# 0xPolygonZero/plonky2

Measured on NVIDIA H100. Metric: goldilocks_field_elements_per_s_ntt_lde_merkle, higher is better.
Workload: dtype u64

## Files before the change

### plonky2_b200/csrc/gl_ntt.cuh

```cuda
#pragma once
#include "gl_lazy.cuh"

namespace gl {

constexpr int NTT_MAX_LOG_PASS = 10;
constexpr int NTT_COL_MIN_LOG = 5;

GL_HD constexpr int ntt_r2(int log) { return log / 2; }
GL_HD constexpr int ntt_r1(int log) { return log - log / 2; }

template <int LOG>
struct PassCfg {
    static constexpr int R1 = ntt_r1(LOG), R2 = ntt_r2(LOG);
    static constexpr int E = 1 << R1, TPT = 1 << R2, NSUB = E / TPT;
    static constexpr int ROW_THREADS = (TPT * 8 < 32) ? 32 : TPT * 8;
    static constexpr int LPC = ROW_THREADS / TPT;
    static constexpr int ROW_MIN_BLOCKS = (E >= 32 ? 512 : 768) / ROW_THREADS;
    static constexpr int ROW_PITCH = TPT + 1;
    static constexpr int ROW_S_WORDS = E * ROW_PITCH;
    static constexpr int GATHER_PITCH = (1 << LOG) + 2;
    static constexpr int T = (256 / TPT) < 8 ? 8 : (256 / TPT);
    static constexpr int COL_THREADS = T * TPT;
    static constexpr int COL_MIN_BLOCKS = (E >= 32 ? 512 : 768) / COL_THREADS;
    static constexpr int COL_QPITCH = TPT * T + 8;
// ... 32 lines not shown
GL_HD void pass_step1(uint64_t* x, const uint64_t* tw, const uint64_t* uq, bool tw_full, int t) {
    using Cf = PassCfg<LOG>;
    L3 r[Cf::E];
#pragma unroll
    for (int q = 0; q < Cf::E; q++) {
        uint64_t v = x[q];
        if (uq && q) v = mul(v, uq[q]);
        r[q] = l3_from(v);
    }
    dft_lazy<Cf::R1>(r);
#pragma unroll
    for (int q = 0; q < Cf::E; q++) {
        uint64_t y = l3_norm(r[q]);
        if (Cf::R2 > 0 && (q || tw_full)) y = mul(y, tw[q * Cf::TPT + t]);
        if (Cf::R2 == 0 && tw_full) y = mul(y, tw[0]);
        x[q] = y;
    }
}
template <int LOG>
GL_HD void pass_step2(uint64_t* z) {
    using Cf = PassCfg<LOG>;
    L3 r[Cf::TPT];
#pragma unroll
    for (int j = 0; j < Cf::TPT; j++) r[j] = l3_from(z[j]);
    dft_lazy<Cf::R2>(r);
#pragma unroll
    for (int j = 0; j < Cf::TPT; j++) z[j] = l3_norm(r[j]);
}

struct ColPass {
    const uint64_t* in;
    uint64_t* out;
    size_t in_stride, out_stride;
    const uint64_t* tw;
    const uint64_t* twa;
    int log_c;
    int log_rb;
    int tw_full;
    int has_uq;
    uint64_t uq[32];
};
template <int LOG>
GL_HD void col_unit(const ColPass& cp, int blk, size_t& in_off, size_t& out_off, int& tile) {
    using Cf = PassCfg<LOG>;
    const int tiles = (1 << cp.log_c) / Cf::T;
    tile = blk % tiles;
    const int unit = blk / tiles;
    const size_t rb = (size_t)unit & (((size_t)1 << cp.log_rb) - 1), col = (size_t)unit >> cp.log_rb;
    const size_t blk_words = (size_t)1 << (LOG + cp.log_c);
    in_off = col * cp.in_stride + rb * blk_words;
    out_off = col * cp.out_stride + rb * blk_words;
}
template <int LOG>
GL_HD void col_load(const ColPass& cp, int blk, int tid, uint64_t* x) {
    using Cf = PassCfg<LOG>;
    const int tt = tid % Cf::T, t = tid / Cf::T;
    size_t in_off, out_off;
    int tile;
    col_unit<LOG>(cp, blk, in_off, out_off, tile);
    const size_t C = (size_t)1 << cp.log_c;
    const uint64_t* src = cp.in + in_off + (size_t)tile * Cf::T + tt;
#pragma unroll
    for (int q = 0; q < Cf::E; q++) x[q] = src[(size_t)(t + Cf::TPT * q) * C];
}
template <int LOG>
GL_HD void col_phase1(const ColPass& cp, uint64_t* S, int blk, int tid, uint64_t* x) {
    using Cf = PassCfg<LOG>;
    const int tt = tid % Cf::T, t = tid / Cf::T;
    size_t in_off, out_off;
    int tile;
    col_unit<LOG>(cp, blk, in_off, out_off, tile);
    const size_t C = (size_t)1 << cp.log_c;
    pass_step1<LOG>(x, cp.tw, cp.has_uq ? cp.uq : nullptr, cp.tw_full != 0, t);
    if (Cf::R2 == 0) {
        uint64_t* dst = cp.out + out_off + (size_t)tile * Cf::T + tt;
        const uint64_t* twa = cp.twa + (size_t)tile * Cf::T + tt;
#pragma unroll
        for (int q = 0; q < Cf::E; q++) dst[(size_t)q * C] = mul(x[q], twa[(size_t)q * C]);
        return;
    }
#pragma unroll
    for (int q = 0; q < Cf::E; q++) S[q * Cf::COL_QPITCH + t * Cf::T + tt] = x[q];
}
template <int LOG>
GL_HD void col_phase2_load(const uint64_t* S, int tid, uint64_t* z ) {
    using Cf = PassCfg<LOG>;
    const int tt = tid % Cf::T, t = tid / Cf::T;
#pragma unroll
    for (int m = 0; m < Cf::NSUB; m++) {
        const int q = t + Cf::TPT * m;
#pragma unroll
        for (int j = 0; j < Cf::TPT; j++) z[m * Cf::TPT + j] = S[q * Cf::COL_QPITCH + j * Cf::T + tt];
    }
}
template <int LOG>
GL_HD void col_phase2_dft(uint64_t* z) {
    using Cf = PassCfg<LOG>;
#pragma unroll
    for (int m = 0; m < Cf::NSUB; m++) pass_step2<LOG>(z + m * Cf::TPT);
}
template <int LOG>
GL_HD int col_twiddle_slot(int tid, int i) { return i * PassCfg<LOG>::COL_THREADS + tid; }
template <int LOG>
GL_HD const uint64_t* col_twiddle_src(const ColPass& cp, int blk, int tid, int i) {
    using Cf = PassCfg<LOG>;
    const int tt = tid % Cf::T, t = tid / Cf::T;
    size_t in_off, out_off;
    int tile;
    col_unit<LOG>(cp, blk, in_off, out_off, tile);
    const int m = i / Cf::TPT, j = i % Cf::TPT;
    const size_t p = (size_t)(t + Cf::TPT * m) * Cf::TPT + j;
    return cp.twa + (p << cp.log_c) + (size_t)tile * Cf::T + tt;
}
template <int LOG>
GL_HD void col_phase2_store(const ColPass& cp, int blk, int tid, const uint64_t* z, const uint64_t* tws, size_t stride_j,
                            size_t stride_m) {
    using Cf = PassCfg<LOG>;
    const int tt = tid % Cf::T, t = tid / Cf::T;
    size_t in_off, out_off;
    int tile;
    col_unit<LOG>(cp, blk, in_off, out_off, tile);
    const size_t C = (size_t)1 << cp.log_c;
    uint64_t* dst = cp.out + out_off + (size_t)tile * Cf::T + tt;
#pragma unroll
    for (int m = 0; m < Cf::NSUB; m++) {
#pragma unroll
        for (int j = 0; j < Cf::TPT; j++) {
            const int i = m * Cf::TPT + j;
            const size_t p = (size_t)(t + Cf::TPT * m) * Cf::TPT + j;
            dst[p * C] = mul(z[i], tws[m * stride_m + j * stride_j]);
        }
    }
}
template <int LOG>
GL_HD void col_phase2(const ColPass& cp, const uint64_t* S, int blk, int tid) {
    using Cf = PassCfg<LOG>;
    if (Cf::R2 == 0) return;
    uint64_t z[Cf::E];
    col_phase2_load<LOG>(S, tid, z);
    col_phase2_dft<LOG>(z);
    const size_t C = (size_t)1 << cp.log_c;
    col_phase2_store<LOG>(cp, blk, tid, z, col_twiddle_src<LOG>(cp, blk, tid, 0), C, (size_t)Cf::TPT * Cf::TPT * C);
}

enum RowMode { RM_BITREV = 0, RM_NATURAL = 1 };
struct RowPass {
    const uint64_t* in;
    uint64_t* out;
    size_t in_stride, out_stride;
    const uint64_t* tw;
    int log_r;
    int ncols;
    int tw_full;
    int has_uq;
    int reverse;
    size_t row0;
    int n_peer;
    uint64_t* out_peer[7];
    uint64_t uq[32];
};
template <int LOG, int MODE>
GL_HD bool row_line(const RowPass& rp, int blk, int l, size_t& col, size_t& prow, size_t& kbase) {
    using Cf = PassCfg<LOG>;
    const size_t L = (size_t)blk * Cf::LPC + l;
    const size_t R = (size_t)1 << rp.log_r;
    col = L >> rp.log_r;
    const size_t low = L & (R - 1);
    if (MODE == RM_BITREV) {
        prow = low;
        kbase = 0;
    } else {
        kbase = low;
        prow = rp.log_r ? (size_t)bitrev32((uint32_t)low, (uint32_t)rp.log_r) : 0;
    }
    return col < (size_t)rp.ncols;
}
template <int LOG>
GL_HD int row_blocks(const RowPass& rp) {
    using Cf = PassCfg<LOG>;
    const size_t lines = (size_t)rp.ncols << rp.log_r;
    return (int)((lines + Cf::LPC - 1) / Cf::LPC);
}
template <int LOG, int MODE>
GL_HD void row_load(const RowPass& rp, int blk, int tid, uint64_t* x) {
    using Cf = PassCfg<LOG>;
    const int l = tid / Cf::TPT, t = tid % Cf::TPT;
    size_t col, prow, kbase;
    const bool live = row_line<LOG, MODE>(rp, blk, l, col, prow, kbase);
    const uint64_t* src = rp.in + col * rp.in_stride + (prow << LOG) + t;
#pragma unroll
    for (int q = 0; q < Cf::E; q++) x[q] = live ? src[Cf::TPT * q] : 0;
}
template <int LOG, int MODE>
GL_HD void row_phase1(const RowPass& rp, uint64_t* S, int blk, int tid, uint64_t* x) {
    using Cf = PassCfg<LOG>;
    const int l = tid / Cf::TPT, t = tid % Cf::TPT;
    pass_step1<LOG>(x, rp.tw, rp.has_uq ? rp.uq : nullptr, rp.tw_full != 0, t);
    if (Cf::R2 == 0) return;
    uint64_t* Sl = S + (size_t)l * Cf::ROW_S_WORDS;
#pragma unroll
    for (int q = 0; q < Cf::E; q++) Sl[q * Cf::ROW_PITCH + t] = x[q];
}
template <int LOG>
GL_HD uint32_t row_natural_index(int q, int j) {
    using Cf = PassCfg<LOG>;
    return bitrev32((uint32_t)q, Cf::R1) + (uint32_t)Cf::E * (Cf::R2 ? bitrev32((uint32_t)j, Cf::R2) : 0u);
}
template <int LOG>
GL_HD void row_phase2_load(const uint64_t* S, int tid, int m, uint64_t* z) {
    using Cf = PassCfg<LOG>;
    const int l = tid / Cf::TPT, t = tid % Cf::TPT;
    const uint64_t* Sl = S + (size_t)l * Cf::ROW_S_WORDS;
    const int q = t + Cf::TPT * m;
#pragma unroll
    for (int j = 0; j < Cf::TPT; j++) z[j] = Sl[q * Cf::ROW_PITCH + j];
}
template <int LOG>
GL_HD void row_store_bitrev(const RowPass& rp, int blk, int tid, int m, const uint64_t* z) {
    using Cf = PassCfg<LOG>;
    const int l = tid / Cf::TPT, t = tid % Cf::TPT;
    size_t col, prow, kbase;
    if (!row_line<LOG, RM_BITREV>(rp, blk, l, col, prow, kbase)) return;
    uint64_t* dst = rp.out + col * rp.out_stride + rp.row0 + (prow << LOG);
    if constexpr (Cf::R2 == 0) {
#pragma unroll
        for (int q = 0; q < Cf::E; q++) dst[q] = canon(z[q]);
    } else {
        const int q = t + Cf::TPT * m;
        uint64_t* d = dst + (size_t)q * Cf::TPT;
#if defined(__CUDA_ARCH__)
#pragma unroll
        for (int j = 0; j < Cf::TPT; j += 2) {
            ulonglong2 v;
            v.x = canon(z[j]);
            v.y = canon(z[j + 1]);
            *reinterpret_cast<ulonglong2*>(d + j) = v;
        }
#else
        for (int j = 0; j < Cf::TPT; j++) d[j] = canon(z[j]);
#endif
    }
}
template <int LOG>
GL_HD void row_gather_write(uint64_t* G, int tid, int m, const uint64_t* z) {
    using Cf = PassCfg<LOG>;
    const int l = tid / Cf::TPT, t = tid % Cf::TPT;
    uint64_t* Gl = G + (size_t)l * Cf::GATHER_PITCH;
    if (Cf::R2 == 0) {
#pragma unroll
        for (int q = 0; q < Cf::E; q++) Gl[row_natural_index<LOG>(q, 0)] = canon(z[q]);
        return;
    }
    const int q = t + Cf::TPT * m;
#pragma unroll
    for (int j = 0; j < Cf::TPT; j++) Gl[row_natural_index<LOG>(q, j)] = canon(z[j]);
}
template <int LOG>
GL_HD void row_store_natural(const RowPass& rp, const uint64_t* G, int blk, int tid, int nthreads) {
    using Cf = PassCfg<LOG>;
    const size_t R = (size_t)1 << rp.log_r, n = R << LOG;
    for (int e = tid; e < Cf::LPC * (1 << LOG); e += nthreads) {
        int l, k2;
        if (rp.log_r) {
            l = e % Cf::LPC;
            k2 = e / Cf::LPC;
        } else {
            k2 = e & ((1 << LOG) - 1);
            l = e >> LOG;
        }
        size_t col, prow, kbase;
        if (!row_line<LOG, RM_NATURAL>(rp, blk, l, col, prow, kbase)) continue;
        size_t k = kbase + ((size_t)k2 << rp.log_r);
        if (rp.reverse) k = (n - k) & (n - 1);
        const uint64_t v = G[(size_t)l * Cf::GATHER_PITCH + k2];
        const size_t at = col * rp.out_stride + k;
        rp.out[at] = v;
        for (int p = 0; p < rp.n_peer; p++) rp.out_peer[p][at] = v;
    }
}

struct NttPlan {
    int a1, a2, b;
};
GL_HD NttPlan ntt_plan(int log_n) {
    NttPlan p{0, 0, log_n};
    if (log_n <= NTT_MAX_LOG_PASS) return p;
    if (log_n <= 2 * NTT_MAX_LOG_PASS) {
        p.b = (log_n + 1) / 2;
        p.a1 = log_n - p.b;
        return p;
    }
    p.b = (log_n + 2) / 3;
    p.a2 = (log_n - p.b + 1) / 2;
    p.a1 = log_n - p.b - p.a2;
    return p;
}


struct TableReq {
    int a, b;
    uint64_t scale, base;
};
struct NttJob {
    NttPlan pl;
    ColPass c1, c2;
    RowPass rp;
    TableReq c1_step, c1_post, c2_step, c2_post, row_step;
};
inline void ntt_make_job(int log_n, NttPlan pl, uint64_t scale, uint64_t shift, NttJob& job) {
    job = NttJob{};
    job.pl = pl;
    const bool coset = canon(shift) != 1;
    const uint64_t one = 1;
    RowPass& rp = job.rp;
    rp.log_r = log_n - pl.b;
    auto fill_uq = [](uint64_t* uq, int log_pass, uint64_t sq) {
        const int E = 1 << ntt_r1(log_pass);
        uint64_t acc = 1;
        for (int q = 0; q < E; q++, acc = mul(acc, sq)) uq[q] = canon(acc);
    };
    if (pl.a1 == 0) {
        job.row_step = TableReq{pl.b, 0, scale, coset ? shift : one};
        rp.tw_full = (canon(scale) != 1 || coset) ? 1 : 0;
        rp.has_uq = coset ? 1 : 0;
        if (coset) fill_uq(rp.uq, pl.b, pow(shift, (uint64_t)1 << ntt_r2(pl.b)));
        return;
    }
    const int c1_log = log_n - pl.a1;
    ColPass& c1 = job.c1;
    c1.log_c = c1_log;
    c1.log_rb = 0;
    job.c1_step = TableReq{pl.a1, 0, one, coset ? pow(shift, (uint64_t)1 << c1_log) : one};
    job.c1_post = TableReq{pl.a1, c1_log, one, coset ? shift : one};
    c1.tw_full = coset ? 1 : 0;
    c1.has_uq = coset ? 1 : 0;
    if (coset) fill_uq(c1.uq, pl.a1, pow(shift, ((uint64_t)1 << ntt_r2(pl.a1)) << c1_log));
    if (pl.a2) {
        ColPass& c2 = job.c2;
        c2.log_c = pl.b;
        c2.log_rb = pl.a1;
        job.c2_step = TableReq{pl.a2, 0, one, one};
        job.c2_post = TableReq{pl.a2, pl.b, one, one};
    }
    job.row_step = TableReq{pl.b, 0, scale, one};
    rp.tw_full = canon(scale) != 1 ? 1 : 0;
}
template <int LOG>
GL_HD int col_blocks(const ColPass& cp, size_t ncols) {
    return (int)((ncols << cp.log_rb) * (((size_t)1 << cp.log_c) / PassCfg<LOG>::T));
}

}
```

### plonky2_b200/csrc/gl_ntt_host.cuh

```cuda
#pragma once

template <int LOG, bool ASYNC_TW>
__global__ void __launch_bounds__(PassCfg<LOG>::COL_THREADS, PassCfg<LOG>::COL_MIN_BLOCKS) k_ntt_col(ColPass cp) {
    using Cf = PassCfg<LOG>;
    extern __shared__ __align__(16) u64 smem[];
    u64* tw_s = smem;
    u64* S = smem + (1 << LOG);
    u64* mbar = S + Cf::COL_S_WORDS;
    tma_table_issue(tw_s, cp.tw, (uint32_t)((1 << LOG) * 8), mbar);
    u64 x[Cf::E];
    col_load<LOG>(cp, blockIdx.x, threadIdx.x, x);
    __syncthreads();
    ColPass c2 = cp;
    c2.tw = tw_s;
    tma_table_wait(mbar);
    col_phase1<LOG>(c2, S, blockIdx.x, threadIdx.x, x);
    if (Cf::R2 == 0) return;
    __syncthreads();
    if (!ASYNC_TW) {
        col_phase2<LOG>(c2, S, blockIdx.x, threadIdx.x);
        return;
    }
    col_phase2_load<LOG>(S, threadIdx.x, x);
    __syncthreads();
#pragma unroll
    for (int i = 0; i < Cf::E; i++) {
        const u64* src = col_twiddle_src<LOG>(cp, blockIdx.x, threadIdx.x, i);
        asm volatile("cp.async.ca.shared.global [%0], [%1], 8;" ::"r"(smem_u32(S + col_twiddle_slot<LOG>(threadIdx.x, i))), "l"(src)
                     : "memory");
    }
    asm volatile("cp.async.commit_group;" ::: "memory");
    col_phase2_dft<LOG>(x);
    asm volatile("cp.async.wait_group 0;" ::: "memory");
    col_phase2_store<LOG>(cp, blockIdx.x, threadIdx.x, x, S + col_twiddle_slot<LOG>(threadIdx.x, 0), Cf::COL_THREADS,
                          (size_t)Cf::TPT * Cf::COL_THREADS);
}

template <int LOG, bool ASYNC_TW>
__global__ void __launch_bounds__(PassCfg<LOG>::COL_THREADS, PassCfg<LOG>::COL_MIN_BLOCKS) k_ntt_col_shared(ColPass cp) {
    using Cf = PassCfg<LOG>;
    static_assert(Cf::E == Cf::TPT, "shared-body column pass needs an even LOG");
    extern __shared__ __align__(16) u64 smem[];
    u64* tw_s = smem;
    u64* S = smem + (1 << LOG);
    u64* mbar = S + Cf::COL_S_WORDS;
    tma_table_issue(tw_s, cp.tw, (uint32_t)((1 << LOG) * 8), mbar);
    u64 x[Cf::E];
    col_load<LOG>(cp, blockIdx.x, threadIdx.x, x);
    __syncthreads();
    tma_table_wait(mbar);
    const int tt = threadIdx.x % Cf::T, t = threadIdx.x / Cf::T;
    size_t in_off, out_off;
    int tile;
    col_unit<LOG>(cp, blockIdx.x, in_off, out_off, tile);
    const size_t C = (size_t)1 << cp.log_c;
    if (cp.has_uq) {
#pragma unroll
        for (int q = 1; q < Cf::E; q++) x[q] = mul(x[q], cp.uq[q]);
    }
    const u64* twp = tw_s + t;
    size_t tws = Cf::TPT;
    bool skip0 = cp.tw_full == 0;
#pragma unroll 1
    for (int s = 0; s < 2; s++) {
        L3 r[Cf::E];
#pragma unroll
        for (int q = 0; q < Cf::E; q++) r[q] = l3_from(x[q]);
        dft_lazy<Cf::R1>(r);
        if (ASYNC_TW && s == 1) asm volatile("cp.async.wait_group 0;" ::: "memory");
#pragma unroll
        for (int q = 0; q < Cf::E; q++) {
            u64 y = l3_norm(r[q]);
            if (!(q == 0 && skip0)) y = mul(y, twp[(size_t)q * tws]);
            x[q] = y;
        }
        if (s == 0) {
#pragma unroll
            for (int q = 0; q < Cf::E; q++) S[q * Cf::COL_QPITCH + t * Cf::T + tt] = x[q];
            __syncthreads();
#pragma unroll
            for (int j = 0; j < Cf::TPT; j++) x[j] = S[t * Cf::COL_QPITCH + j * Cf::T + tt];
            skip0 = false;
            const u64* tw2 = cp.twa + (((size_t)t * Cf::TPT) << cp.log_c) + (size_t)tile * Cf::T + tt;
            if (ASYNC_TW) {
                __syncthreads();
#pragma unroll
                for (int j = 0; j < Cf::TPT; j++)
                    asm volatile("cp.async.ca.shared.global [%0], [%1], 8;" ::"r"(smem_u32(S + col_twiddle_slot<LOG>(threadIdx.x, j))),
                                 "l"(tw2 + (size_t)j * C)
                                 : "memory");
                asm volatile("cp.async.commit_group;" ::: "memory");
                twp = S + col_twiddle_slot<LOG>(threadIdx.x, 0);
                tws = Cf::COL_THREADS;
            } else {
                twp = tw2;
                tws = C;
            }
        }
    }
    u64* dst = cp.out + out_off + (size_t)tile * Cf::T + tt;
#pragma unroll
    for (int j = 0; j < Cf::TPT; j++) dst[((size_t)t * Cf::TPT + j) * C] = x[j];
}

template <int LOG, int MODE>
__global__ void __launch_bounds__(PassCfg<LOG>::ROW_THREADS, PassCfg<LOG>::ROW_MIN_BLOCKS) k_ntt_row(RowPass rp) {
    using Cf = PassCfg<LOG>;
    extern __shared__ __align__(16) u64 smem[];
    u64* tw_s = smem;
    u64* S = smem + (1 << LOG);
    u64* mbar = S + ntt_row_smem_bytes(LOG, MODE == RM_NATURAL) / 8;
    RowPass r2 = rp;
    u64 x[Cf::E];
    if (Cf::R2 > 0 && LOG >= 4) {
        tma_table_issue(tw_s, rp.tw, (uint32_t)((1 << LOG) * 8), mbar);
        row_load<LOG, MODE>(rp, blockIdx.x, threadIdx.x, x);
        __syncthreads();
        r2.tw = tw_s;
        tma_table_wait(mbar);
    } else {
        row_load<LOG, MODE>(rp, blockIdx.x, threadIdx.x, x);
    }
    row_phase1<LOG, MODE>(r2, S, blockIdx.x, threadIdx.x, x);
    if (Cf::R2 == 0) {
        if (MODE == RM_BITREV) {
            row_store_bitrev<LOG>(r2, blockIdx.x, threadIdx.x, 0, x);
        } else {
            row_gather_write<LOG>(S, threadIdx.x, 0, x);
            __syncthreads();
            row_store_natural<LOG>(r2, S, blockIdx.x, threadIdx.x, blockDim.x);
        }
        return;
    }
    __syncwarp();
    if (MODE == RM_BITREV) {
#pragma unroll
        for (int m = 0; m < Cf::NSUB; m++) {
            u64 z[Cf::TPT];
            row_phase2_load<LOG>(S, threadIdx.x, m, z);
            pass_step2<LOG>(z);
            row_store_bitrev<LOG>(r2, blockIdx.x, threadIdx.x, m, z);
        }
    } else {
        u64 z[Cf::NSUB][Cf::TPT];
#pragma unroll
        for (int m = 0; m < Cf::NSUB; m++) {
            row_phase2_load<LOG>(S, threadIdx.x, m, z[m]);
            pass_step2<LOG>(z[m]);
        }
        __syncthreads();
#pragma unroll
        for (int m = 0; m < Cf::NSUB; m++) row_gather_write<LOG>(S, threadIdx.x, m, z[m]);
        __syncthreads();
        row_store_natural<LOG>(r2, S, blockIdx.x, threadIdx.x, blockDim.x);
    }
}

template <int LOG, int MODE>
__global__ void __launch_bounds__(PassCfg<LOG>::ROW_THREADS, PassCfg<LOG>::ROW_MIN_BLOCKS) k_ntt_row_shared(RowPass rp) {
    using Cf = PassCfg<LOG>;
    static_assert(Cf::E == Cf::TPT && Cf::R2 > 0 && LOG >= 4, "shared-body row pass needs an even LOG >= 4");
    extern __shared__ __align__(16) u64 smem[];
    u64* tw_s = smem;
    u64* S = smem + (1 << LOG);
    u64* mbar = S + ntt_row_smem_bytes(LOG, MODE == RM_NATURAL) / 8;
    u64 x[Cf::E];
    tma_table_issue(tw_s, rp.tw, (uint32_t)((1 << LOG) * 8), mbar);
    row_load<LOG, MODE>(rp, blockIdx.x, threadIdx.x, x);
    __syncthreads();
    tma_table_wait(mbar);
    const int l = threadIdx.x / Cf::TPT, t = threadIdx.x % Cf::TPT;
    u64* Sl = S + (size_t)l * Cf::ROW_S_WORDS;
    if (rp.has_uq) {
#pragma unroll
        for (int q = 1; q < Cf::E; q++) x[q] = mul(x[q], rp.uq[q]);
    }
    const bool skip0 = rp.tw_full == 0;
    bool do_mul = true;
#pragma unroll 1
    for (int s = 0; s < 2; s++) {
        L3 r[Cf::E];
#pragma unroll
        for (int q = 0; q < Cf::E; q++) r[q] = l3_from(x[q]);
        dft_lazy<Cf::R1>(r);
#pragma unroll
        for (int q = 0; q < Cf::E; q++) {
            u64 y = l3_norm(r[q]);
            if (do_mul && !(q == 0 && skip0)) y = mul(y, tw_s[q * Cf::TPT + t]);
            x[q] = y;
        }
        if (s == 0) {
#pragma unroll
            for (int q = 0; q < Cf::E; q++) Sl[q * Cf::ROW_PITCH + t] = x[q];
            __syncwarp();
#pragma unroll
            for (int j = 0; j < Cf::TPT; j++) x[j] = Sl[t * Cf::ROW_PITCH + j];
            do_mul = false;
        }
    }
    if (MODE == RM_BITREV) {
        row_store_bitrev<LOG>(rp, blockIdx.x, threadIdx.x, 0, x);
    } else {
        __syncthreads();
        row_gather_write<LOG>(S, threadIdx.x, 0, x);
        __syncthreads();
        row_store_natural<LOG>(rp, S, blockIdx.x, threadIdx.x, blockDim.x);
    }
}

__global__ void k_fill_step(int log, u64 scale, u64 base, u64* out) {
    uint32_t j = blockIdx.x * blockDim.x + threadIdx.x;
    if (j < (1u << log)) out[j] = table_step_entry(log, j, scale, base);
}
__global__ void k_fill_post(int a, int b, u64 base, u64* out) {
    size_t i = (size_t)blockIdx.x * blockDim.x + threadIdx.x;
    if (i < ((size_t)1 << (a + b))) out[i] = table_post_entry(a, b, i, base);
}
__global__ void k_fill_pows(const u64* bases, int ntab, size_t count, u64* out) {
    size_t i = (size_t)blockIdx.x * blockDim.x + threadIdx.x;
    if (i >= count * ntab) return;
    size_t t = i / count, e = i % count;
    out[i] = gl::pow(bases[t], e);
}
__global__ void k_mul_pows(u64* data, size_t stride, size_t n, const u64* hi, const u64* lo, int lowbits) {
    size_t k = (size_t)blockIdx.x * blockDim.x + threadIdx.x;
    if (k >= n) return;
    u64* col = data + (size_t)blockIdx.y * stride;
    u64 f = mul(hi[k >> lowbits], lo[k & (((size_t)1 << lowbits) - 1)]);
    col[k] = canon(mul(col[k], f));
}

template <int LOG>
static int launch_col(gl_ctx* ctx, const ColPass& cp, size_t ncols) {
    const int nblocks = col_blocks<LOG>(cp, ncols);
    const size_t smem = ((size_t)(1 << LOG) + PassCfg<LOG>::COL_S_WORDS) * 8 + 16;
    auto go = [&](auto kern) -> int {
        const void* fn = (const void*)kern;
        if (!ctx->smem_attr_done.count(fn)) {
            CK(ctx, cudaFuncSetAttribute(kern, cudaFuncAttributeMaxDynamicSharedMemorySize, (int)smem));
            CK(ctx, cudaFuncSetAttribute(kern, cudaFuncAttributePreferredSharedMemoryCarveout, cudaSharedmemCarveoutMaxShared));
            ctx->smem_attr_done.insert(fn);
        }
        kern<<<nblocks, PassCfg<LOG>::COL_THREADS, smem, ctx->stream>>>(cp);
        CKL(ctx);
        return GL_OK;
    };
    if constexpr (PassCfg<LOG>::E == PassCfg<LOG>::TPT) {
        if (ctx->ntt_variant == 0) return cp.has_uq ? go(k_ntt_col_shared<LOG, true>) : go(k_ntt_col_shared<LOG, false>);
    }
    return cp.has_uq ? go(k_ntt_col<LOG, true>) : go(k_ntt_col<LOG, false>);
}
template <int LOG, int MODE>
static int launch_row(gl_ctx* ctx, const RowPass& rp) {
    const size_t smem = (size_t)(1 << LOG) * 8 + ntt_row_smem_bytes(LOG, MODE == RM_NATURAL) + 16;
    auto go = [&](auto kern) -> int {
        const void* fn = (const void*)kern;
        if (!ctx->smem_attr_done.count(fn)) {
            CK(ctx, cudaFuncSetAttribute(kern, cudaFuncAttributeMaxDynamicSharedMemorySize, (int)smem));
            CK(ctx, cudaFuncSetAttribute(kern, cudaFuncAttributePreferredSharedMemoryCarveout, cudaSharedmemCarveoutMaxShared));
            ctx->smem_attr_done.insert(fn);
        }
        kern<<<row_blocks<LOG>(rp), PassCfg<LOG>::ROW_THREADS, smem, ctx->stream>>>(rp);
        CKL(ctx);
        return GL_OK;
    };
    if constexpr (PassCfg<LOG>::E == PassCfg<LOG>::TPT && LOG >= 4) {
        if (ctx->ntt_variant == 0) return go(k_ntt_row_shared<LOG, MODE>);
    }
    return go(k_ntt_row<LOG, MODE>);
}
static int dispatch_col(gl_ctx* ctx, int a, const ColPass& cp, size_t ncols) {
    switch (a) {
        case 5: return launch_col<5>(ctx, cp, ncols);
        case 6: return launch_col<6>(ctx, cp, ncols);
        case 7: return launch_col<7>(ctx, cp, ncols);
        case 8: return launch_col<8>(ctx, cp, ncols);
        case 9: return launch_col<9>(ctx, cp, ncols);
        case 10: return launch_col<10>(ctx, cp, ncols);
    }
    return set_err(ctx, GL_ERR_UNSUPPORTED, "column pass log %d", a);
}
static int dispatch_row(gl_ctx* ctx, int b, int mode, const RowPass& rp) {
#define ROW_CASE(L)                                                     \
    case L:                                                             \
        return mode == RM_BITREV ? launch_row<L, RM_BITREV>(ctx, rp) : launch_row<L, RM_NATURAL>(ctx, rp);
    switch (b) {
        ROW_CASE(1) ROW_CASE(2) ROW_CASE(3) ROW_CASE(4) ROW_CASE(5) ROW_CASE(6) ROW_CASE(7) ROW_CASE(8) ROW_CASE(9) ROW_CASE(10)
    }
#undef ROW_CASE
    return set_err(ctx, GL_ERR_UNSUPPORTED, "row pass log %d", b);
}

static void table_cache_trim(gl_ctx* ctx, size_t incoming_bytes) {
    const size_t cap = (size_t)3 << 30;
    if (ctx->table_bytes + incoming_bytes <= cap) return;
    for (auto& kv : ctx->step_tabs) cudaFreeAsync(kv.second, ctx->stream);
    for (auto& kv : ctx->post_tabs) cudaFreeAsync(kv.second, ctx->stream);
    ctx->step_tabs.clear();
    ctx->post_tabs.clear();
    ctx->table_bytes = 0;
}
static int get_step(gl_ctx* ctx, int log, u64 scale, u64 base, const u64** out) {
    auto key = std::make_tuple(log, canon(scale), canon(base));
    auto it = ctx->step_tabs.find(key);
    if (it == ctx->step_tabs.end()) {
        const size_t words = ((size_t)1 << log) < 2 ? 2 : ((size_t)1 << log);
        DevBuf p(ctx);
        TRY(p.alloc(words));
        k_fill_step<<<((1 << log) + 255) / 256, 256, 0, ctx->stream>>>(log, canon(scale), canon(base), p.get());
        CKL(ctx);
        ctx->table_bytes += words * 8;
        it = ctx->step_tabs.emplace(key, p.release()).first;
    }
    *out = it->second;
    return GL_OK;
}
static int get_post(gl_ctx* ctx, int a, int b, u64 base, const u64** out) {
    auto key = std::make_tuple(a, b, canon(base));
    auto it = ctx->post_tabs.find(key);
    if (it == ctx->post_tabs.end()) {
        const size_t words = (size_t)1 << (a + b);
        DevBuf p(ctx);
        TRY(p.alloc(words));
        k_fill_post<<<(unsigned)((words + 255) / 256), 256, 0, ctx->stream>>>(a, b, canon(base), p.get());
        CKL(ctx);
        ctx->table_bytes += words * 8;
        it = ctx->post_tabs.emplace(key, p.release()).first;
    }
    *out = it->second;
    return GL_OK;
}
static uint32_t group_cols(const gl_ctx* ctx, int log_n, uint32_t ncols) {
    uint32_t g = ctx->ntt_group;
    if (g == 0) {
        size_t col_bytes = (size_t)8 << log_n;
        size_t target = (size_t)1 << 30;
        g = (uint32_t)(target / col_bytes);
        if (g < 8) g = 8;
    }
    g = (g + 7) & ~7u;
    if (g > ((ncols + 7) & ~7u)) g = (ncols + 7) & ~7u;
    return g;
}

static int build_pow_tables(gl_ctx* ctx, const std::vector<u64>& bases, size_t count, DevBuf& out) {
    const int ntab = (int)bases.size();
    DevBuf dbases(ctx);
    TRY(dbases.alloc(ntab));
    TRY(h2d(ctx, dbases.get(), bases.data(), ntab));
    TRY(out.alloc(count * ntab));
    size_t total = count * ntab;
    k_fill_pows<<<(unsigned)((total + 255) / 256), 256, 0, ctx->stream>>>(dbases.get(), ntab, count, out.get());
    CKL(ctx);
    return GL_OK;
}

struct PeerOuts {
    int n = 0;
    u64* p[7] = {nullptr, nullptr, nullptr, nullptr, nullptr, nullptr, nullptr};
};
static int ntt_forward(gl_ctx* ctx, const u64* in, size_t in_stride, u64* out, size_t out_stride, size_t row0, int log_n,
                       uint32_t ncols, int mode, bool reverse, u64 scale, u64 shift, const PeerOuts* peers = nullptr) {
    if (ncols == 0) return GL_OK;
    if (log_n < 1 || log_n > 3 * NTT_MAX_LOG_PASS) return set_err(ctx, GL_ERR_UNSUPPORTED, "log_n %d not in 1..30", log_n);
    const NttPlan pl = ntt_plan(log_n);
    const size_t n = (size_t)1 << log_n;
    table_cache_trim(ctx, 2 * n * 8 + (1 << 16));
    NttJob job;
    ntt_make_job(log_n, pl, scale, shift, job);
    RowPass& rp = job.rp;
    rp.out_stride = out_stride;
    rp.reverse = reverse ? 1 : 0;
    rp.row0 = row0;
    rp.n_peer = peers ? peers->n : 0;
    for (int i = 0; i < rp.n_peer; i++) rp.out_peer[i] = peers->p[i];
    TRY(get_step(ctx, job.row_step.a, job.row_step.scale, job.row_step.base, &rp.tw));
    if (pl.a1 == 0) {
        rp.in = in;
        rp.in_stride = in_stride;
        rp.out = out;
        rp.ncols = (int)ncols;
        return dispatch_row(ctx, pl.b, mode, rp);
    }
    const uint32_t G = group_cols(ctx, log_n, ncols);
    TRY(ensure_scratch(ctx, (size_t)G * n));
    ColPass &c1 = job.c1, &c2 = job.c2;
    c1.out = ctx->scratch;
    c1.in_stride = in_stride;
    c1.out_stride = n;
    TRY(get_step(ctx, job.c1_step.a, job.c1_step.scale, job.c1_step.base, &c1.tw));
    TRY(get_post(ctx, job.c1_post.a, job.c1_post.b, job.c1_post.base, &c1.twa));
    if (pl.a2) {
        c2.in = c2.out = ctx->scratch;
// ... 22 lines not shown
}

static int ntt_natural(gl_ctx* ctx, const u64* in, size_t in_stride, u64* out, size_t out_stride, int log_n,
                       uint32_t ncols, bool inverse, u64 shift, const PeerOuts* peers = nullptr) {
    if (ncols == 0) return GL_OK;
    const size_t n = (size_t)1 << log_n;
    if (peers && peers->n && (log_n == 0 || canon(shift) != 1))
        return set_err(ctx, GL_ERR_UNSUPPORTED, "multi-destination transforms need log_n >= 1 and no coset shift");
    if (log_n == 0) {
        if (in != out)
            CK(ctx, cudaMemcpy2DAsync(out, out_stride * 8, in, in_stride * 8, 8, ncols, cudaMemcpyDeviceToDevice,
                                      ctx->stream));
        k_scale1<<<(ncols + 127) / 128, 128, 0, ctx->stream>>>(out, out_stride, ncols, 1);
        CKL(ctx);
        return GL_OK;
    }
    if (!inverse) return ntt_forward(ctx, in, in_stride, out, out_stride, 0, log_n, ncols, RM_NATURAL, false, 1, shift, peers);
    TRY(ntt_forward(ctx, in, in_stride, out, out_stride, 0, log_n, ncols, RM_NATURAL, true, inverse_2exp((uint32_t)log_n), 1,
                    peers));
    if (canon(shift) != 1) {
        const int lowbits = log_n > 12 ? 12 : log_n;
        const size_t lo_cnt = (size_t)1 << lowbits, hi_cnt = (size_t)1 << (log_n - lowbits);
        const u64 sinv = gl::inv(shift);
        const size_t tcnt = lo_cnt > hi_cnt ? lo_cnt : hi_cnt;
        DevBuf tabs(ctx);
        TRY(build_pow_tables(ctx, std::vector<u64>{gl::pow(sinv, lo_cnt), sinv}, tcnt, tabs));
        for (uint32_t b0 = 0; b0 < ncols; b0 += MAX_GRID_Y) {
            const uint32_t bc = (ncols - b0 < MAX_GRID_Y) ? ncols - b0 : MAX_GRID_Y;
            k_mul_pows<<<dim3((unsigned)((n + 255) / 256), bc), 256, 0, ctx->stream>>>(
                out + (size_t)b0 * out_stride, out_stride, n, tabs.get(), tabs.get() + tcnt, lowbits);
            CKL(ctx);
        }
    }
    return GL_OK;
}

__global__ void k_lde_const(const u64* coeffs, size_t stride, uint32_t ncols, int ncos, u64* lde, size_t lde_stride) {
    uint32_t i = blockIdx.x * blockDim.x + threadIdx.x;
    if (i >= ncols * (uint32_t)ncos) return;
    uint32_t col = i / ncos, c = i % ncos;
    lde[(size_t)col * lde_stride + c] = canon(coeffs[(size_t)col * stride]);
}

static int lde_columns(gl_ctx* ctx, const u64* coeffs, size_t coeff_stride, uint32_t ncols, int log_n, int rate_bits,
                       u64 base_shift, u64* lde, size_t lde_stride) {
    if (ncols == 0) return GL_OK;
    const size_t n = (size_t)1 << log_n;
    const int ncos = 1 << rate_bits;
    if (log_n == 0) {
        k_lde_const<<<(ncols * ncos + 127) / 128, 128, 0, ctx->stream>>>(coeffs, coeff_stride, ncols, ncos, lde, lde_stride);
        CKL(ctx);
        return GL_OK;
    }
    const u64 wN = root_of_unity((uint32_t)(log_n + rate_bits));
    const uint32_t G = log_n > NTT_MAX_LOG_PASS ? group_cols(ctx, log_n, ncols) : ncols;
    for (uint32_t g0 = 0; g0 < ncols; g0 += G) {
        const uint32_t gc = (ncols - g0 < G) ? ncols - g0 : G;
        for (int c = 0; c < ncos; c++) {
            const u64 s = mul(base_shift, gl::pow(wN, bitrev32((uint32_t)c, (uint32_t)rate_bits)));
            TRY(ntt_forward(ctx, coeffs + (size_t)g0 * coeff_stride, coeff_stride, lde + (size_t)g0 * lde_stride, lde_stride,
                            (size_t)c * n, log_n, gc, RM_BITREV, false, 1, s));
        }
    }
    return GL_OK;
}
```

### plonky2_b200/csrc/plonky2_b200.cu

```cuda
#include <cooperative_groups.h>
#include <cub/device/device_radix_sort.cuh>
#include <cuda_runtime.h>

#include <cstdarg>
#include <cstdio>
#include <cstring>
#include <functional>
#include <initializer_list>
#include <map>
#include <memory>
#include <set>
#include <string>
#include <tuple>
#include <vector>

#include <sys/random.h>

#include <cerrno>

#include "../../include/plonky2_b200.h"
#include "gl_chacha.cuh"
#include "gl_field.cuh"
#include "gl_logup.cuh"
#include "gl_ctl.cuh"
#include "gl_ntt.cuh"
#include "gl_poseidon.cuh"
#include "gl_sigma.cuh"
#include "gl_vanishing.cuh"

using namespace gl;
typedef uint64_t u64;

static thread_local std::string g_last_error;

struct gl_ctx {
    int device = 0;
    cudaStream_t stream = nullptr;
    bool own_stream = false;
    u64 launches = 0;
    std::string err;
    std::map<std::tuple<int, u64, u64>, u64*> step_tabs;
    std::map<std::tuple<int, int, u64>, u64*> post_tabs;
    size_t table_bytes = 0;
    std::map<int, u64*> fold_tabs;
    cudaStream_t copy_stream = nullptr;
    std::set<const void*> smem_attr_done;
    u64* scratch = nullptr;
    size_t scratch_words = 0;
    u64* pinned = nullptr;
    size_t pinned_words = 0;
    u64* dstage = nullptr;
    size_t dstage_words = 0;
    uint32_t ntt_group = 0;
    int ntt_variant = 0;
    int sm_count = 0;
    int coop_ok = 0;
    int coop_blocks_per_sm = 0;
    bool prof_on = false;
    struct Pending {
        int phase;
        cudaEvent_t a, b;
    };
    std::vector<Pending> prof_pending;
    double prof_ms[GL_NUM_PHASES] = {0};
    u64 prof_count[GL_NUM_PHASES] = {0};
};

struct PhaseScope {
    gl_ctx* ctx;
    cudaEvent_t a = nullptr, b = nullptr;
    int phase;
    PhaseScope(gl_ctx* c, int ph) : ctx(c), phase(ph) {
        if (!ctx->prof_on) return;
        cudaEventCreate(&a);
        cudaEventCreate(&b);
        cudaEventRecord(a, ctx->stream);
    }
    ~PhaseScope() {
        if (!a) return;
        cudaEventRecord(b, ctx->stream);
        ctx->prof_pending.push_back({phase, a, b});
    }
};

static int set_err(gl_ctx* ctx, int code, const char* fmt, ...) {
    char buf[512];
    va_list ap;
    va_start(ap, fmt);
    vsnprintf(buf, sizeof(buf), fmt, ap);
    va_end(ap);
    g_last_error = buf;
    if (ctx) ctx->err = buf;
    return code;
}
#define CK(ctx, call)                                                                          \
    do {                                                                                       \
        cudaError_t e_ = (call);                                                               \
        if (e_ != cudaSuccess)                                                                 \
            return set_err(ctx, e_ == cudaErrorMemoryAllocation ? GL_ERR_OOM : GL_ERR_CUDA,    \
                           "%s failed: %s", #call, cudaGetErrorString(e_));                    \
    } while (0)
#define CKL(ctx)                                                                               \
    do {                                                                                       \
        (ctx)->launches++;                                                                     \
        cudaError_t e_ = cudaGetLastError();                                                   \
        if (e_ != cudaSuccess)                                                                 \
            return set_err(ctx, GL_ERR_CUDA, "kernel launch failed (%s:%d): %s", __FILE__,     \
// ... 1408 lines not shown
    if (rc_init != GL_OK) {
        if (ctx->own_stream) cudaStreamDestroy(ctx->stream);
        delete ctx;
        return rc_init;
    }
    cudaMemPool_t pool;
    if (cudaDeviceGetDefaultMemPool(&pool, device) == cudaSuccess) {
        unsigned long long thr = ~0ULL;
        cudaMemPoolSetAttribute(pool, cudaMemPoolAttrReleaseThreshold, &thr);
    }
    *out = ctx;
    return GL_OK;
}
void gl_ctx_destroy(gl_ctx* ctx) {
    if (!ctx) return;
    cudaSetDevice(ctx->device);
    cudaStreamSynchronize(ctx->stream);
    for (auto& kv : ctx->step_tabs) cudaFreeAsync(kv.second, ctx->stream);
    for (auto& kv : ctx->post_tabs) cudaFreeAsync(kv.second, ctx->stream);
    for (auto& kv : ctx->fold_tabs) cudaFreeAsync(kv.second, ctx->stream);
    if (ctx->copy_stream) cudaStreamDestroy(ctx->copy_stream);
    if (ctx->scratch) cudaFreeAsync(ctx->scratch, ctx->stream);
    if (ctx->dstage) cudaFreeAsync(ctx->dstage, ctx->stream);
    if (ctx->pinned) cudaFreeHost(ctx->pinned);
    cudaStreamSynchronize(ctx->stream);
    if (ctx->own_stream) cudaStreamDestroy(ctx->stream);
    delete ctx;
}
const char* gl_last_error(const gl_ctx* ctx) { return ctx ? ctx->err.c_str() : g_last_error.c_str(); }
int gl_ctx_synchronize(gl_ctx* ctx) {
    CK(ctx, cudaStreamSynchronize(ctx->stream));
    return GL_OK;
}
int gl_ctx_device_bytes(gl_ctx* ctx, uint64_t* in_use, uint64_t* high, int reset_high) {
    if (!ctx) return set_err(ctx, GL_ERR_BAD_ARG, "null context");
    CK(ctx, cudaSetDevice(ctx->device));
    CK(ctx, cudaStreamSynchronize(ctx->stream));
    cudaMemPool_t pool;
    CK(ctx, cudaDeviceGetDefaultMemPool(&pool, ctx->device));
    uint64_t v = 0;
    CK(ctx, cudaMemPoolGetAttribute(pool, cudaMemPoolAttrUsedMemCurrent, &v));
    if (in_use) *in_use = v;
    CK(ctx, cudaMemPoolGetAttribute(pool, cudaMemPoolAttrUsedMemHigh, &v));
    if (high) *high = v;
    if (reset_high) {
        uint64_t zero = 0;
        CK(ctx, cudaMemPoolSetAttribute(pool, cudaMemPoolAttrUsedMemHigh, &zero));
    }
    return GL_OK;
}
uint64_t gl_ctx_launch_count(const gl_ctx* ctx) { return ctx->launches; }
int gl_ctx_set_ntt_group(gl_ctx* ctx, uint32_t columns) {
    ctx->ntt_variant = (columns >> 31) & 1;
    ctx->ntt_group = columns & 0x7FFFFFFFu;
    return GL_OK;
}
int gl_ctx_set_profiling(gl_ctx* ctx, int on) {
    ctx->prof_on = on != 0;
    return GL_OK;
}
int gl_ctx_phase_ms(gl_ctx* ctx, int phase, double* ms, uint64_t* count) {
    if (phase < 0 || phase >= GL_NUM_PHASES) return set_err(ctx, GL_ERR_BAD_ARG, "bad phase");
    if (!ctx->prof_pending.empty()) {
        CK(ctx, cudaStreamSynchronize(ctx->stream));
        for (auto& p : ctx->prof_pending) {
            float t = 0;
            cudaEventElapsedTime(&t, p.a, p.b);
            ctx->prof_ms[p.phase] += t;
            ctx->prof_count[p.phase]++;
            cudaEventDestroy(p.a);
            cudaEventDestroy(p.b);
        }
        ctx->prof_pending.clear();
    }
    if (ms) *ms = ctx->prof_ms[phase];
    if (count) *count = ctx->prof_count[phase];
    return GL_OK;
}
int gl_ctx_reset_phases(gl_ctx* ctx) {
    TRY(gl_ctx_phase_ms(ctx, 0, nullptr, nullptr));
    for (int i = 0; i < GL_NUM_PHASES; i++) {
        ctx->prof_ms[i] = 0;
        ctx->prof_count[i] = 0;
    }
    return GL_OK;
}

int gl_ntt(gl_ctx* ctx, uint64_t* data, uint32_t log_n, uint32_t batch, size_t stride, int inverse,
           uint32_t zero_factor_log, uint64_t coset_shift, int mem) {
    (void)zero_factor_log;
    if (!ctx || !data) return set_err(ctx, GL_ERR_BAD_ARG, "null argument");
    CK(ctx, cudaSetDevice(ctx->device));
    if (log_n > 3 * NTT_MAX_LOG_PASS) return set_err(ctx, GL_ERR_UNSUPPORTED, "log_n %u > 30", log_n);
    const size_t n = (size_t)1 << log_n;
    if (batch > 1 && stride < n) return set_err(ctx, GL_ERR_BAD_SHAPE, "stride %zu < n %zu", stride, n);
    if (canon(coset_shift) == 0) return set_err(ctx, GL_ERR_BAD_ARG, "coset_shift must be non-zero");
    if (mem == GL_MEM_DEVICE) return ntt_natural(ctx, data, stride, data, stride, (int)log_n, batch, inverse != 0, coset_shift);
    DevBuf d(ctx);
    TRY(d.alloc((size_t)batch * n));
    const size_t pitch = (batch > 1 ? stride : n) * 8;
    if (cudaMemcpy2DAsync(d.get(), n * 8, data, pitch, n * 8, batch, cudaMemcpyHostToDevice, ctx->stream) != cudaSuccess)
        return set_err(ctx, GL_ERR_CUDA, "H2D: %s", cudaGetErrorString(cudaGetLastError()));
    TRY(ntt_natural(ctx, d.get(), n, d.get(), n, (int)log_n, batch, inverse != 0, coset_shift));
    cudaError_t e = cudaMemcpy2DAsync(data, pitch, d.get(), n * 8, n * 8, batch, cudaMemcpyDeviceToHost, ctx->stream);
    if (e != cudaSuccess) return set_err(ctx, GL_ERR_CUDA, "D2H: %s", cudaGetErrorString(e));
    if (cudaStreamSynchronize(ctx->stream) != cudaSuccess)
        return set_err(ctx, GL_ERR_CUDA, "sync failed: %s", cudaGetErrorString(cudaGetLastError()));
// ... 1654 lines not shown
```

Measured before the change: 8.046 billion.

## Batch multiple LDE cosets per column pass and stage bitrev row stores via shared memory

Adds a coset-batched column NTT kernel that reads each coefficient column once and produces up to eight coset outputs per launch, each coset with its own twiddle and scaling tables. The batched path then runs the remaining column and row passes over all cosets together, writing to per-coset offsets. The aim is to cut repeated coefficient reads and the per-coset launch overhead. The bit-reversed row store is also changed to stage results in shared memory first so that global writes are coalesced. In exchange it needs more scratch memory and table cache space, and the column group size is divided by the number of cosets.

```diff
diff --git a/plonky2_b200/csrc/gl_ntt.cuh b/plonky2_b200/csrc/gl_ntt.cuh
--- a/plonky2_b200/csrc/gl_ntt.cuh
+++ b/plonky2_b200/csrc/gl_ntt.cuh
@@ -108,16 +108,43 @@
     out_off = col * cp.out_stride + rb * blk_words;
 }
 template <int LOG>
+GL_HD void col_load_at(const ColPass& cp, size_t in_off, int tile, int tid, uint64_t* x) {
+    using Cf = PassCfg<LOG>;
+    const int tt = tid % Cf::T, t = tid / Cf::T;
+    const size_t C = (size_t)1 << cp.log_c;
+    const uint64_t* src = cp.in + in_off + (size_t)tile * Cf::T + tt;
+#pragma unroll
+    for (int q = 0; q < Cf::E; q++) x[q] = src[(size_t)(t + Cf::TPT * q) * C];
+}
+template <int LOG>
 GL_HD void col_load(const ColPass& cp, int blk, int tid, uint64_t* x) {
-    using Cf = PassCfg<LOG>;
-    const int tt = tid % Cf::T, t = tid / Cf::T;
     size_t in_off, out_off;
     int tile;
     col_unit<LOG>(cp, blk, in_off, out_off, tile);
-    const size_t C = (size_t)1 << cp.log_c;
-    const uint64_t* src = cp.in + in_off + (size_t)tile * Cf::T + tt;
-#pragma unroll
-    for (int q = 0; q < Cf::E; q++) x[q] = src[(size_t)(t + Cf::TPT * q) * C];
+    col_load_at<LOG>(cp, in_off, tile, tid, x);
+}
+
+constexpr int COL_LOG_MAX_COSETS = 3;
+struct ColCosets {
+    ColPass cp;
+    int log_cos;
+    int ncols;
+    const uint64_t* tw[1 << COL_LOG_MAX_COSETS];
+    const uint64_t* twa[1 << COL_LOG_MAX_COSETS];
+    uint64_t uq[1 << COL_LOG_MAX_COSETS][32];
+};
+template <int LOG>
+GL_HD void col_cosets_unit(const ColCosets& cc, int blk, int& c, size_t& in_off, size_t& out_off, int& tile) {
+    c = blk & ((1 << cc.log_cos) - 1);
+    const int rest = blk >> cc.log_cos;
+    const size_t col = (size_t)(rest % cc.ncols);
+    tile = rest / cc.ncols;
+    in_off = col * cc.cp.in_stride;
+    out_off = ((col << cc.log_cos) + c) * cc.cp.out_stride;
+}
+template <int LOG>
+GL_HD int col_cosets_blocks(const ColCosets& cc) {
+    return (cc.ncols << cc.log_cos) * (int)(((size_t)1 << cc.cp.log_c) / PassCfg<LOG>::T);
 }
 template <int LOG>
 GL_HD void col_phase1(const ColPass& cp, uint64_t* S, int blk, int tid, uint64_t* x) {
@@ -211,6 +238,8 @@
     int has_uq;
     int reverse;
     size_t row0;
+    int log_cos;
+    size_t cos_step;
     int n_peer;
     uint64_t* out_peer[7];
     uint64_t uq[32];
@@ -272,12 +301,17 @@
     for (int j = 0; j < Cf::TPT; j++) z[j] = Sl[q * Cf::ROW_PITCH + j];
 }
 template <int LOG>
+GL_HD uint64_t* row_bitrev_dst(const RowPass& rp, size_t col, size_t prow) {
+    const size_t cos = col & (((size_t)1 << rp.log_cos) - 1);
+    return rp.out + (col >> rp.log_cos) * rp.out_stride + rp.row0 + cos * rp.cos_step + (prow << LOG);
+}
+template <int LOG>
 GL_HD void row_store_bitrev(const RowPass& rp, int blk, int tid, int m, const uint64_t* z) {
     using Cf = PassCfg<LOG>;
     const int l = tid / Cf::TPT, t = tid % Cf::TPT;
     size_t col, prow, kbase;
     if (!row_line<LOG, RM_BITREV>(rp, blk, l, col, prow, kbase)) return;
-    uint64_t* dst = rp.out + col * rp.out_stride + rp.row0 + (prow << LOG);
+    uint64_t* dst = row_bitrev_dst<LOG>(rp, col, prow);
     if constexpr (Cf::R2 == 0) {
 #pragma unroll
         for (int q = 0; q < Cf::E; q++) dst[q] = canon(z[q]);
@@ -296,6 +330,26 @@
         for (int j = 0; j < Cf::TPT; j++) d[j] = canon(z[j]);
 #endif
     }
+}
+template <int LOG>
+GL_HD void row_stage_bitrev(uint64_t* S, int tid, const uint64_t* z) {
+    using Cf = PassCfg<LOG>;
+    static_assert(Cf::E == Cf::TPT, "one step-2 transform per thread");
+    const int l = tid / Cf::TPT, t = tid % Cf::TPT;
+    uint64_t* Sl = S + (size_t)l * Cf::ROW_S_WORDS;
+#pragma unroll
+    for (int j = 0; j < Cf::TPT; j++) Sl[t * Cf::ROW_PITCH + j] = canon(z[j]);
+}
+template <int LOG>
+GL_HD void row_store_bitrev_staged(const RowPass& rp, const uint64_t* S, int blk, int tid) {
+    using Cf = PassCfg<LOG>;
+    const int l = tid / Cf::TPT, t = tid % Cf::TPT;
+    size_t col, prow, kbase;
+    if (!row_line<LOG, RM_BITREV>(rp, blk, l, col, prow, kbase)) return;
+    uint64_t* dst = row_bitrev_dst<LOG>(rp, col, prow) + t;
+    const uint64_t* Sl = S + (size_t)l * Cf::ROW_S_WORDS + t;
+#pragma unroll
+    for (int k = 0; k < Cf::E; k++) dst[(size_t)k * Cf::TPT] = Sl[k * Cf::ROW_PITCH];
 }
 template <int LOG>
 GL_HD void row_gather_write(uint64_t* G, int tid, int m, const uint64_t* z) {
@@ -401,6 +455,24 @@
     job.row_step = TableReq{pl.b, 0, scale, one};
     rp.tw_full = canon(scale) != 1 ? 1 : 0;
 }
+inline void lde_make_cosets_job(int log_n, NttPlan pl, int rate_bits, uint64_t base_shift, int c0, int log_kc,
+                                NttJob& job, ColCosets& cc, TableReq* steps, TableReq* posts) {
+    const uint64_t wN = root_of_unity((uint32_t)(log_n + rate_bits));
+    cc = ColCosets{};
+    for (int c = 0; c < (1 << log_kc); c++) {
+        const uint64_t s = mul(base_shift, pow(wN, bitrev32((uint32_t)(c0 + c), (uint32_t)rate_bits)));
+        NttJob jc;
+        ntt_make_job(log_n, pl, 1, s, jc);
+        if (c == 0) job = jc;
+        steps[c] = jc.c1_step;
+        posts[c] = jc.c1_post;
+        for (int q = 0; q < 32; q++) cc.uq[c][q] = jc.c1.has_uq ? jc.c1.uq[q] : 1;
+    }
+    cc.cp = job.c1;
+    cc.cp.has_uq = cc.cp.tw_full = 1;
+    cc.log_cos = log_kc;
+    job.rp.log_cos = log_kc;
+}
 template <int LOG>
 GL_HD int col_blocks(const ColPass& cp, size_t ncols) {
     return (int)((ncols << cp.log_rb) * (((size_t)1 << cp.log_c) / PassCfg<LOG>::T));
diff --git a/plonky2_b200/csrc/gl_ntt_host.cuh b/plonky2_b200/csrc/gl_ntt_host.cuh
--- a/plonky2_b200/csrc/gl_ntt_host.cuh
+++ b/plonky2_b200/csrc/gl_ntt_host.cuh
@@ -37,26 +37,24 @@
 }
 
 template <int LOG, bool ASYNC_TW>
-__global__ void __launch_bounds__(PassCfg<LOG>::COL_THREADS, PassCfg<LOG>::COL_MIN_BLOCKS) k_ntt_col_shared(ColPass cp) {
+__device__ __forceinline__ void col_shared_body(const ColPass& cp, const u64* tw, const u64* twa, const u64 (&uq)[32],
+                                                size_t in_off, size_t out_off, int tile) {
     using Cf = PassCfg<LOG>;
     static_assert(Cf::E == Cf::TPT, "shared-body column pass needs an even LOG");
     extern __shared__ __align__(16) u64 smem[];
     u64* tw_s = smem;
     u64* S = smem + (1 << LOG);
     u64* mbar = S + Cf::COL_S_WORDS;
-    tma_table_issue(tw_s, cp.tw, (uint32_t)((1 << LOG) * 8), mbar);
+    tma_table_issue(tw_s, tw, (uint32_t)((1 << LOG) * 8), mbar);
     u64 x[Cf::E];
-    col_load<LOG>(cp, blockIdx.x, threadIdx.x, x);
+    col_load_at<LOG>(cp, in_off, tile, threadIdx.x, x);
     __syncthreads();
     tma_table_wait(mbar);
     const int tt = threadIdx.x % Cf::T, t = threadIdx.x / Cf::T;
-    size_t in_off, out_off;
-    int tile;
-    col_unit<LOG>(cp, blockIdx.x, in_off, out_off, tile);
     const size_t C = (size_t)1 << cp.log_c;
     if (cp.has_uq) {
 #pragma unroll
-        for (int q = 1; q < Cf::E; q++) x[q] = mul(x[q], cp.uq[q]);
+        for (int q = 1; q < Cf::E; q++) x[q] = mul(x[q], uq[q]);
     }
     const u64* twp = tw_s + t;
     size_t tws = Cf::TPT;
@@ -81,7 +79,7 @@
 #pragma unroll
             for (int j = 0; j < Cf::TPT; j++) x[j] = S[t * Cf::COL_QPITCH + j * Cf::T + tt];
             skip0 = false;
-            const u64* tw2 = cp.twa + (((size_t)t * Cf::TPT) << cp.log_c) + (size_t)tile * Cf::T + tt;
+            const u64* tw2 = twa + (((size_t)t * Cf::TPT) << cp.log_c) + (size_t)tile * Cf::T + tt;
             if (ASYNC_TW) {
                 __syncthreads();
 #pragma unroll
@@ -101,6 +99,20 @@
     u64* dst = cp.out + out_off + (size_t)tile * Cf::T + tt;
 #pragma unroll
     for (int j = 0; j < Cf::TPT; j++) dst[((size_t)t * Cf::TPT + j) * C] = x[j];
+}
+template <int LOG, bool ASYNC_TW>
+__global__ void __launch_bounds__(PassCfg<LOG>::COL_THREADS, PassCfg<LOG>::COL_MIN_BLOCKS) k_ntt_col_shared(ColPass cp) {
+    size_t in_off, out_off;
+    int tile;
+    col_unit<LOG>(cp, blockIdx.x, in_off, out_off, tile);
+    col_shared_body<LOG, ASYNC_TW>(cp, cp.tw, cp.twa, cp.uq, in_off, out_off, tile);
+}
+template <int LOG>
+__global__ void __launch_bounds__(PassCfg<LOG>::COL_THREADS, PassCfg<LOG>::COL_MIN_BLOCKS) k_ntt_col_cosets(ColCosets cc) {
+    size_t in_off, out_off;
+    int c, tile;
+    col_cosets_unit<LOG>(cc, blockIdx.x, c, in_off, out_off, tile);
+    col_shared_body<LOG, true>(cc.cp, cc.tw[c], cc.twa[c], cc.uq[c], in_off, out_off, tile);
 }
 
 template <int LOG, int MODE>
@@ -199,7 +211,10 @@
         }
     }
     if (MODE == RM_BITREV) {
-        row_store_bitrev<LOG>(rp, blockIdx.x, threadIdx.x, 0, x);
+        __syncwarp();
+        row_stage_bitrev<LOG>(S, threadIdx.x, x);
+        __syncwarp();
+        row_store_bitrev_staged<LOG>(rp, S, blockIdx.x, threadIdx.x);
     } else {
         __syncthreads();
         row_gather_write<LOG>(S, threadIdx.x, 0, x);
@@ -279,6 +294,29 @@
         case 10: return launch_col<10>(ctx, cp, ncols);
     }
     return set_err(ctx, GL_ERR_UNSUPPORTED, "column pass log %d", a);
+}
+template <int LOG>
+static int launch_col_cosets(gl_ctx* ctx, const ColCosets& cc) {
+    const size_t smem = ((size_t)(1 << LOG) + PassCfg<LOG>::COL_S_WORDS) * 8 + 16;
+    auto kern = k_ntt_col_cosets<LOG>;
+    const void* fn = (const void*)kern;
+    if (!ctx->smem_attr_done.count(fn)) {
+        CK(ctx, cudaFuncSetAttribute(kern, cudaFuncAttributeMaxDynamicSharedMemorySize, (int)smem));
+        CK(ctx, cudaFuncSetAttribute(kern, cudaFuncAttributePreferredSharedMemoryCarveout, cudaSharedmemCarveoutMaxShared));
+        ctx->smem_attr_done.insert(fn);
+    }
+    kern<<<col_cosets_blocks<LOG>(cc), PassCfg<LOG>::COL_THREADS, smem, ctx->stream>>>(cc);
+    CKL(ctx);
+    return GL_OK;
+}
+static bool col_cosets_supported(int a) { return a == 6 || a == 8 || a == 10; }
+static int dispatch_col_cosets(gl_ctx* ctx, int a, const ColCosets& cc) {
+    switch (a) {
+        case 6: return launch_col_cosets<6>(ctx, cc);
+        case 8: return launch_col_cosets<8>(ctx, cc);
+        case 10: return launch_col_cosets<10>(ctx, cc);
+    }
+    return set_err(ctx, GL_ERR_UNSUPPORTED, "coset column pass log %d", a);
 }
 static int dispatch_row(gl_ctx* ctx, int b, int mode, const RowPass& rp) {
 #define ROW_CASE(L)                                                     \
@@ -330,7 +368,7 @@
     *out = it->second;
     return GL_OK;
 }
-static uint32_t group_cols(const gl_ctx* ctx, int log_n, uint32_t ncols) {
+static uint32_t group_cols(const gl_ctx* ctx, int log_n, uint32_t ncols, uint32_t cosets = 1) {
     uint32_t g = ctx->ntt_group;
     if (g == 0) {
         size_t col_bytes = (size_t)8 << log_n;
@@ -339,6 +377,10 @@
         if (g < 8) g = 8;
     }
     g = (g + 7) & ~7u;
+    if (cosets > 1) {
+        g = g / cosets ? g / cosets : 1;
+        return g < ncols ? g : ncols;
+    }
     if (g > ((ncols + 7) & ~7u)) g = (ncols + 7) & ~7u;
     return g;
 }
@@ -467,6 +509,51 @@
         CKL(ctx);
         return GL_OK;
     }
+    const NttPlan pl = ntt_plan(log_n);
+    if (ncos > 1 && pl.a1 && col_cosets_supported(pl.a1) && ctx->ntt_variant == 0 && !ctx->lde_per_coset) {
+        const int log_kc = rate_bits < COL_LOG_MAX_COSETS ? rate_bits : COL_LOG_MAX_COSETS, kc = 1 << log_kc;
+        const uint32_t G = group_cols(ctx, log_n, ncols, kc);
+        TRY(ensure_scratch(ctx, (size_t)G * kc * n));
+        for (uint32_t g0 = 0; g0 < ncols; g0 += G) {
+            const uint32_t gc = (ncols - g0 < G) ? ncols - g0 : G;
+            for (int c0 = 0; c0 < ncos; c0 += kc) {
+                table_cache_trim(ctx, (size_t)(kc + 1) * (n * 8 + (1 << 16)));
+                NttJob job;
+                ColCosets cc;
+                TableReq steps[1 << COL_LOG_MAX_COSETS], posts[1 << COL_LOG_MAX_COSETS];
+                lde_make_cosets_job(log_n, pl, rate_bits, base_shift, c0, log_kc, job, cc, steps, posts);
+                for (int c = 0; c < kc; c++) {
+                    TRY(get_step(ctx, steps[c].a, steps[c].scale, steps[c].base, &cc.tw[c]));
+                    TRY(get_post(ctx, posts[c].a, posts[c].b, posts[c].base, &cc.twa[c]));
+                }
+                cc.cp.in = coeffs + (size_t)g0 * coeff_stride;
+                cc.cp.in_stride = coeff_stride;
+                cc.cp.out = ctx->scratch;
+                cc.cp.out_stride = n;
+                cc.ncols = (int)gc;
+                TRY(dispatch_col_cosets(ctx, pl.a1, cc));
+                if (pl.a2) {
+                    ColPass& c2 = job.c2;
+                    c2.in = c2.out = ctx->scratch;
+                    c2.in_stride = c2.out_stride = n;
+                    TRY(get_step(ctx, job.c2_step.a, job.c2_step.scale, job.c2_step.base, &c2.tw));
+                    TRY(get_post(ctx, job.c2_post.a, job.c2_post.b, job.c2_post.base, &c2.twa));
+                    TRY(dispatch_col(ctx, pl.a2, c2, (size_t)gc * kc));
+                }
+                RowPass& rp = job.rp;
+                TRY(get_step(ctx, job.row_step.a, job.row_step.scale, job.row_step.base, &rp.tw));
+                rp.in = ctx->scratch;
+                rp.in_stride = n;
+                rp.out = lde + (size_t)g0 * lde_stride;
+                rp.out_stride = lde_stride;
+                rp.row0 = (size_t)c0 * n;
+                rp.cos_step = n;
+                rp.ncols = (int)(gc * kc);
+                TRY(dispatch_row(ctx, pl.b, RM_BITREV, rp));
+            }
+        }
+        return GL_OK;
+    }
     const u64 wN = root_of_unity((uint32_t)(log_n + rate_bits));
     const uint32_t G = log_n > NTT_MAX_LOG_PASS ? group_cols(ctx, log_n, ncols) : ncols;
     for (uint32_t g0 = 0; g0 < ncols; g0 += G) {
diff --git a/plonky2_b200/csrc/plonky2_b200.cu b/plonky2_b200/csrc/plonky2_b200.cu
--- a/plonky2_b200/csrc/plonky2_b200.cu
+++ b/plonky2_b200/csrc/plonky2_b200.cu
@@ -53,6 +53,7 @@
     size_t dstage_words = 0;
     uint32_t ntt_group = 0;
     int ntt_variant = 0;
+    bool lde_per_coset = false;
     int sm_count = 0;
     int coop_ok = 0;
     int coop_blocks_per_sm = 0;
@@ -1567,7 +1568,8 @@
 uint64_t gl_ctx_launch_count(const gl_ctx* ctx) { return ctx->launches; }
 int gl_ctx_set_ntt_group(gl_ctx* ctx, uint32_t columns) {
     ctx->ntt_variant = (columns >> 31) & 1;
-    ctx->ntt_group = columns & 0x7FFFFFFFu;
+    ctx->lde_per_coset = (columns >> 30) & 1;
+    ctx->ntt_group = columns & 0x3FFFFFFFu;
     return GL_OK;
 }
 int gl_ctx_set_profiling(gl_ctx* ctx, int on) {
```

Result: faster. 8.490 billion, median of 6 (+5.5%).
